# huj31415/nbody3d-webgpu

Hardware: AMD Instinct MI355X
Metric: pair-interactions/s (higher is better)
Workload: dtype f32; 1 GPU; N=262144 Plummer sphere, dt=1e-3, G=1, eps2=1e-4, i-sharded over 1 GPU(s); n=262144, kernel_variant=f32pk_symw_ipl16_j1_w2048_r32t128, parallelism=1gpu

## Files before the change

### include/nbody3d_hip.h

```cpp
#ifndef NBODY3D_HIP_H
#define NBODY3D_HIP_H

#include <stddef.h>
#include <stdint.h>

#ifdef __cplusplus
extern "C" {
#endif
#if defined(__GNUC__)
#pragma GCC visibility push(default)
#endif

#define NB_ABI_VERSION 2u
#define NB_ABI_MINOR 4u

typedef struct nb_sim nb_sim;

typedef enum nb_status {
    NB_OK = 0,
    NB_ERR_INVALID = 1,
    NB_ERR_NO_DEVICE = 2,
    NB_ERR_HIP = 3,
    NB_ERR_STATE = 4,
    NB_ERR_NOMEM = 5,
    NB_ERR_COMM = 6,
    NB_NOT_READY = 7
} nb_status;

typedef enum nb_precision { NB_F32 = 0, NB_F64 = 1 } nb_precision;

#define NB_FLAG_EXT_STREAM 1u
#define NB_FLAG_LDS_ONLY 4u
#define NB_FLAG_NO_FUSE 8u
#define NB_FLAG_POISON 16u

#define NB_FLAG_JPK_FENCED 32u

#define NB_FLAG_NO_SYM 64u

#define NB_FLAG_SYM_SHARD 128u

#define NB_FLAG_WHOLE_SWEEPS 256u

typedef enum nb_array { NB_BODIES = 0, NB_VEL = 1, NB_ACCEL = 2 } nb_array;

typedef struct nb_config {
    uint32_t struct_size;
    uint32_t n;
    uint32_t precision;
    uint32_t tile;
    double eps2;
    int32_t device;
    uint32_t shard_begin;
    uint32_t shard_count;
    void *ext_stream;
    void *ext_bodies;
    uint32_t force_variant;
    uint32_t jsplit;
    uint32_t flags;
    uint32_t layer_budget_mib;
    uint32_t reserved[4];
} nb_config;

uint32_t nb_abi_version(void);
uint32_t nb_abi_minor(void);

int nb_device_count(void);

int nb_create(const nb_config *cfg, nb_sim **out);

void nb_destroy(nb_sim *s);

int nb_upload(nb_sim *s, const void *bodies, const void *vel, const void *accel);

int nb_set_params(nb_sim *s, double dt, double G);

int nb_step(nb_sim *s, uint32_t nsteps);

int nb_download(nb_sim *s, void *bodies, void *vel, void *accel);

int nb_sync(nb_sim *s);

const char *nb_last_error(nb_sim *s);


int nb_device_ptr(nb_sim *s, int which , void **out);

typedef int (*nb_exchange_fn)(void *user, void *bodies_dev, size_t elem_size,
                              uint32_t n, uint32_t shard_begin,
                              uint32_t shard_count, void *hip_stream);
int nb_set_exchange(nb_sim *s, nb_exchange_fn fn, void *user);

typedef int (*nb_exchange_wait_fn)(void *user, void *hip_stream);
int nb_set_exchange_overlapped(nb_sim *s, nb_exchange_fn begin, nb_exchange_wait_fn wait, void *user);

// ... 80 lines not shown
```

### nbody3d-webgpu_amd/csrc/kernels/symmetric.hip.h

```cpp
#pragma once

namespace nb {

template <typename T> struct SymRowT { T x, y, z; };
using SymRow = SymRowT<float>;

constexpr uint32_t kFlushSteps = 4096;

template <int NG>
__device__ __forceinline__ void flush_resident_sums(float (*hi)[64], const int lane, const bool flushed, nb_f2 (&ax)[NG], nb_f2 (&ay)[NG], nb_f2 (&az)[NG])
{
    if (flushed) {
#pragma unroll
        for (int c = 0; c < NG; ++c) {
            hi[6 * c + 0][lane] += ax[c].x; hi[6 * c + 1][lane] += ay[c].x; hi[6 * c + 2][lane] += az[c].x;
            hi[6 * c + 3][lane] += ax[c].y; hi[6 * c + 4][lane] += ay[c].y; hi[6 * c + 5][lane] += az[c].y;
        }
    } else {
#pragma unroll
        for (int c = 0; c < NG; ++c) {
            hi[6 * c + 0][lane] = ax[c].x; hi[6 * c + 1][lane] = ay[c].x; hi[6 * c + 2][lane] = az[c].x;
            hi[6 * c + 3][lane] = ax[c].y; hi[6 * c + 4][lane] = ay[c].y; hi[6 * c + 5][lane] = az[c].y;
        }
    }
#pragma unroll
    for (int c = 0; c < NG; ++c) { ax[c] = nb_f2{0, 0}; ay[c] = nb_f2{0, 0}; az[c] = nb_f2{0, 0}; }
}

__device__ __forceinline__ float wave_rot1(float v)
{
    const int iv = __builtin_bit_cast(int, v);
    return __builtin_bit_cast(float, __builtin_amdgcn_update_dpp(iv, iv, 0x13C , 0xF, 0xF, false));
}

template <int WS, int NG, int J>
__global__ __launch_bounds__(64 * WS) __attribute__((amdgpu_waves_per_eu(NG > 4 ? 2 : 4, NG > 4 ? 2 : 4)))
void nb_force_sym(const float4* __restrict__ bodies, SymRow* __restrict__ partial, const SymPlan pl, const uint32_t n, const float eps2)
{
    constexpr uint32_t RB = 128u * NG;
    constexpr uint32_t S = RB * WS;
    constexpr uint32_t CH = 64u * J;
    constexpr uint32_t CPS = S / CH;
    __shared__ float red[WS > 1 ? 2 : 1][WS > 1 ? WS : 1][3 * J][64];
    const int tid = threadIdx.x;
    const int lane = tid & 63;
    const uint32_t w = __builtin_amdgcn_readfirstlane(tid >> 6);

    const uint32_t g = blockIdx.x / pl.q, q = blockIdx.x % pl.q;
    const uint32_t ring = (pl.H + (g < pl.n_hi ? 1u : 0u)) * CPS;
    const uint32_t total = ring + CPS;
    const uint32_t c0 = (uint32_t)(((uint64_t)q * total) / pl.q), c1 = (uint32_t)(((uint64_t)(q + 1) * total) / pl.q);

    nb_f2 xi[NG], yi[NG], zi[NG], mi[NG], ax[NG], ay[NG], az[NG];
    {
        const float4* rb = bodies + (size_t)g * S + w * RB + lane;
#pragma unroll
        for (int c = 0; c < NG; ++c) {
            const float4 b0 = ld4(rb + (2 * c) * 64), b1 = ld4(rb + (2 * c + 1) * 64);
            xi[c] = nb_f2{b0.x, b1.x}; yi[c] = nb_f2{b0.y, b1.y}; zi[c] = nb_f2{b0.z, b1.z}; mi[c] = nb_f2{b0.w, b1.w};
            ax[c] = nb_f2{0, 0}; ay[c] = nb_f2{0, 0}; az[c] = nb_f2{0, 0};
        }
    }
    const nb_f2 e2 = nb_f2{eps2, eps2};

    uint32_t done = 0;
    for (uint32_t k = c0; k < c1; ++k) {
        const bool sym = k < ring;
        const uint32_t d = k / CPS;
        uint32_t tb = g + 1 + d;
        if (tb >= pl.nsb) tb -= pl.nsb;
        const uint32_t tstart = sym ? tb * S + (k % CPS) * CH : g * S + (k - ring) * CH;
        if (tstart >= n) continue;
        float tx[J], ty[J], tz[J], tm[J];
        nb_f2 bx[J], by[J], bz[J];
#pragma unroll
        for (int u = 0; u < J; ++u) {
            const float4 t = ld4(bodies + tstart + u * 64 + lane);
            tx[u] = t.x; ty[u] = t.y; tz[u] = t.z; tm[u] = t.w;
            bx[u] = nb_f2{0, 0}; by[u] = nb_f2{0, 0}; bz[u] = nb_f2{0, 0};
        }
        for (int st = 0; st < 64; ++st) {
#pragma unroll
            for (int u = 0; u < J; ++u) {
                const nb_f2 px = nb_f2{tx[u], tx[u]}, py = nb_f2{ty[u], ty[u]}, pz = nb_f2{tz[u], tz[u]}, pm = nb_f2{tm[u], tm[u]};
#pragma unroll
// ... 53 lines not shown
#pragma unroll
                for (int u = 0; u < J; ++u) {
                    red[buf][w][3 * u + 0][lane] = bx[u].x + bx[u].y;
                    red[buf][w][3 * u + 1][lane] = by[u].x + by[u].y;
                    red[buf][w][3 * u + 2][lane] = bz[u].x + bz[u].y;
                }
                __syncthreads();
                if (w == done % WS) {
#pragma unroll
                    for (int u = 0; u < J; ++u) {
                        float sx = red[buf][0][3 * u + 0][lane], sy = red[buf][0][3 * u + 1][lane], sz = red[buf][0][3 * u + 2][lane];
#pragma unroll
                        for (int ww = 1; ww < WS; ++ww) { sx += red[buf][ww][3 * u + 0][lane]; sy += red[buf][ww][3 * u + 1][lane]; sz += red[buf][ww][3 * u + 2][lane]; }
                        out[u * 64] = SymRow{sx, sy, sz};
                    }
                }
            }
        }
    }
    SymRow* out = partial + (size_t)(pl.r_layer0 + q) * pl.np + (size_t)g * S + w * RB + lane;
#pragma unroll
    for (int c = 0; c < NG; ++c) {
        out[(2 * c) * 64] = SymRow{ax[c].x, ay[c].x, az[c].x};
        out[(2 * c + 1) * 64] = SymRow{ax[c].y, ay[c].y, az[c].y};
    }
}

struct SymWK { uint32_t np, nsb, W, total_hi, total_lo, n_hi, zc, ups, r_layer0, t_layer0; };
#define SYMW_PLAN_PARAMS const uint32_t W_, const uint32_t ups_, const uint32_t nsb_, const uint32_t zc_, const uint32_t r_layer0_, const uint32_t t_layer0_
typedef uint32_t nb_u4 __attribute__((ext_vector_type(4)));
template <int TAIL>
__device__ __forceinline__ void symw_record_and_tail(const uint32_t* rec_at, nb_u4& rec, uint32_t (&tail)[TAIL])
{
    static_assert(TAIL == 1 || TAIL == 4, "f32: eps2; f64: G, eps2");
    constexpr int kTailOffset = 4 * 8 + 6 * 4;
    if constexpr (TAIL == 1) {
        asm volatile("s_load_dwordx4 %0, %2, 0x0\n\ts_load_dword %1, %3, %4\n\ts_waitcnt lgkmcnt(0)"
                     : "=&s"(rec), "=&s"(tail[0]) : "s"(rec_at), "s"(__builtin_amdgcn_kernarg_segment_ptr()), "n"(kTailOffset) : "memory");
    } else {
        nb_u4 t;
        asm volatile("s_load_dwordx4 %0, %2, 0x0\n\ts_load_dwordx4 %1, %3, %4\n\ts_waitcnt lgkmcnt(0)"
                     : "=&s"(rec), "=&s"(t) : "s"(rec_at), "s"(__builtin_amdgcn_kernarg_segment_ptr()), "n"(kTailOffset) : "memory");
        tail[0] = t.x; tail[1] = t.y; tail[2] = t.z; tail[3] = t.w;
    }
}

__device__ __forceinline__ SymWK symw_plan_words(uint32_t S, uint32_t cps, uint32_t W, uint32_t ups, uint32_t nsb, uint32_t zc, uint32_t r_layer0, uint32_t t_layer0)
{
    const uint32_t H = (nsb - 1u) >> 1, n_hi = (nsb & 1u) ? 0u : nsb >> 1;
    const uint32_t total_lo = (H + 1u) * cps + zc, total_hi = total_lo + (n_hi ? cps : 0u);
    return SymWK{(nsb + (zc ? 1u : 0u)) * S, nsb, W, total_hi, total_lo, n_hi, zc, ups, r_layer0, t_layer0};
}

template <int NG, int J>
__global__ __launch_bounds__(256) __attribute__((amdgpu_waves_per_eu(NG >= 4 ? 2 : 4, NG > 4 ? 2 : (NG < 4 ? 8 : 4))))
void nb_force_symw(const uint32_t* __restrict__ gtab, const float4* __restrict__ bodies, SymRow* __restrict__ partial, SymRow* __restrict__ spill,
                   SYMW_PLAN_PARAMS, const float eps2_arg ,
                   uint32_t* __restrict__ queue, const uint32_t npieces, const uint32_t pieces_off)
{
    constexpr uint32_t S = 128u * NG;
    constexpr int GW = NG < 4 ? NG : 4;
    constexpr uint32_t CH = 64u * J;
    constexpr uint32_t CPS = S / CH;
    const SymWK pl = symw_plan_words(S, CPS, W_, ups_, nsb_, zc_, r_layer0_, t_layer0_);
    const int lane = threadIdx.x & 63, wi = threadIdx.x >> 6;
    const uint32_t w = __builtin_amdgcn_readfirstlane(blockIdx.x * 4u + wi);
    const bool active = w < pl.W;
    NB_STAMP(0);
    __shared__ float red[4][6 * NG][64];
    __shared__ uint32_t fin[4];
    const uint32_t ups = pl.ups, ush = (uint32_t)__builtin_ctz(ups), ustep = 64u >> ush,
                   tab1 = 2u * (pl.np / S);
    nb_u4 rec;
    uint32_t tail[1];
    symw_record_and_tail(gtab + tab1 + 4u * (active ? w : 0u), rec, tail);
    const float eps2 = __builtin_bit_cast(float, tail[0]);
    const nb_f2 e2 = nb_f2{eps2, eps2};
    const uint32_t first_lo = pl.n_hi * pl.total_hi, first_z = first_lo + (pl.nsb - pl.n_hi) * pl.total_lo;
    const uint32_t slot = rec.w;
    NB_STAMP_LIGHT(1);
    bool first_part = true;

    auto run = [&](uint32_t u, const uint32_t uend, const uint32_t piece_layer) -> uint32_t {
        uint32_t gfin = ~0u;
        while (u < uend) {
            const uint32_t p = u >> ush;
            uint32_t g, k, total;
            if (p < first_lo) { g = p / pl.total_hi; k = p - g * pl.total_hi; total = pl.total_hi; }
            else if (p < first_z) { const uint32_t r = p - first_lo; g = pl.n_hi + r / pl.total_lo; k = r - (g - pl.n_hi) * pl.total_lo; total = pl.total_lo; }
            else { g = pl.nsb; k = p - first_z; total = pl.zc; }
            const uint32_t ring = g < pl.nsb ? total - CPS - pl.zc : 0u;
            const uint32_t both_end = g < pl.nsb ? ring + pl.zc : 0u;
            uint32_t ug_end = (p - k + total) * ups;
            if (ug_end > uend) ug_end = uend;

            nb_f2 xi[NG], yi[NG], zi[NG], mi[NG], ax[NG], ay[NG], az[NG];
            {
                const float4* rb = bodies + (size_t)g * S + lane;
#pragma unroll
                for (int c = 0; c < NG; ++c) {
                    const float4 b0 = ld4(rb + (2 * c) * 64), b1 = ld4(rb + (2 * c + 1) * 64);
                    xi[c] = nb_f2{b0.x, b1.x}; yi[c] = nb_f2{b0.y, b1.y}; zi[c] = nb_f2{b0.z, b1.z}; mi[c] = nb_f2{b0.w, b1.w};
                    ax[c] = nb_f2{0, 0}; ay[c] = nb_f2{0, 0}; az[c] = nb_f2{0, 0};
                }
            }
            uint32_t since = 0;
            bool flushed = false;
            while (u < ug_end) {
                const uint32_t q0 = u & (ups - 1u);
                uint32_t nun = ups - q0;
                if (nun > ug_end - u) nun = ug_end - u;
                const uint32_t s0 = q0 * ustep, s1 = s0 + nun * ustep;
                u += nun;
                if (since >= kFlushSteps) {
                    flush_resident_sums<NG>(red[wi], lane, flushed, ax, ay, az);
                    flushed = true;
                    since = 0;
                }
                since += s1 - s0;
                const bool sym = k < both_end, zsweep = k >= ring && sym;
                const uint32_t d = k / CPS;
                uint32_t tb = g + 1 + d;
                if (tb >= pl.nsb) tb -= pl.nsb;
                const uint32_t tstart = k < ring ? tb * S + (k % CPS) * CH : zsweep ? pl.nsb * S + (k - ring) * CH : g * S + (k - both_end) * CH;
                const uint32_t zrow = g * pl.zc + (k - ring);
                ++k;
                float tx[J], ty[J], tz[J], tm[J];
                nb_f2 bx[J], by[J], bz[J];
                const uint32_t src = ((uint32_t)lane - s0) & 63u;
#pragma unroll
                for (int uu = 0; uu < J; ++uu) {
                    const float4 t = ld4(bodies + tstart + uu * 64 + src);
                    tx[uu] = t.x; ty[uu] = t.y; tz[uu] = t.z; tm[uu] = t.w;
                    bx[uu] = nb_f2{0, 0}; by[uu] = nb_f2{0, 0}; bz[uu] = nb_f2{0, 0};
                }
                auto steps = [&](auto both) {
                    constexpr bool BOTH = decltype(both)::value;
                    for (uint32_t st = s0; st < s1; ++st) {
#pragma unroll
                        for (int uu = 0; uu < J; ++uu) {
                            const nb_f2 px = nb_f2{tx[uu], tx[uu]}, py = nb_f2{ty[uu], ty[uu]}, pz = nb_f2{tz[uu], tz[uu]}, pm = nb_f2{tm[uu], tm[uu]};
#pragma unroll
                            for (int c0g = 0; c0g < NG; c0g += GW) {
                                nb_f2 dx[GW], dy[GW], dz[GW], d2[GW], r[GW], si[GW], sj[GW];
#pragma unroll
                                for (int c = 0; c < GW; ++c) dx[c] = px - xi[c0g + c];
#pragma unroll
                                for (int c = 0; c < GW; ++c) dy[c] = py - yi[c0g + c];
#pragma unroll
                                for (int c = 0; c < GW; ++c) dz[c] = pz - zi[c0g + c];
#pragma unroll
                                for (int c = 0; c < GW; ++c) d2[c] = __builtin_elementwise_fma(dx[c], dx[c], e2);
#pragma unroll
                                for (int c = 0; c < GW; ++c) d2[c] = __builtin_elementwise_fma(dy[c], dy[c], d2[c]);
#pragma unroll
                                for (int c = 0; c < GW; ++c) d2[c] = __builtin_elementwise_fma(dz[c], dz[c], d2[c]);
#pragma unroll
                                for (int c = 0; c < GW; ++c) r[c] = d2[c] * d2[c];
#pragma unroll
                                for (int c = 0; c < GW; ++c) r[c] = r[c] * d2[c];
#pragma unroll
                                for (int c = 0; c < GW; ++c) r[c] = nb_f2{nb_rsq(r[c].x), nb_rsq(r[c].y)};
#pragma unroll
                                for (int c = 0; c < GW; ++c) si[c] = pm * r[c];
                                if constexpr (BOTH) {
#pragma unroll
                                    for (int c = 0; c < GW; ++c) sj[c] = mi[c0g + c] * r[c];
                                }
#pragma unroll
                                for (int c = 0; c < GW; ++c) ax[c0g + c] = __builtin_elementwise_fma(si[c], dx[c], ax[c0g + c]);
#pragma unroll
                                for (int c = 0; c < GW; ++c) ay[c0g + c] = __builtin_elementwise_fma(si[c], dy[c], ay[c0g + c]);
#pragma unroll
                                for (int c = 0; c < GW; ++c) az[c0g + c] = __builtin_elementwise_fma(si[c], dz[c], az[c0g + c]);
                                if constexpr (BOTH) {
#pragma unroll
                                    for (int c = 0; c < GW; ++c) bx[uu] = __builtin_elementwise_fma(-sj[c], dx[c], bx[uu]);
#pragma unroll
                                    for (int c = 0; c < GW; ++c) by[uu] = __builtin_elementwise_fma(-sj[c], dy[c], by[uu]);
// ... 45 lines not shown
                        ax[c].y += red[wi][6 * c + 3][lane]; ay[c].y += red[wi][6 * c + 4][lane]; az[c].y += red[wi][6 * c + 5][lane];
                    }
                    red[wi][6 * c + 0][lane] = ax[c].x; red[wi][6 * c + 1][lane] = ay[c].x; red[wi][6 * c + 2][lane] = az[c].x;
                    red[wi][6 * c + 3][lane] = ax[c].y; red[wi][6 * c + 4][lane] = ay[c].y; red[wi][6 * c + 5][lane] = az[c].y;
                }
                break;
            }
            SymRow* out = partial + (size_t)(pl.r_layer0 + gtab[2 * g + 1] - 1u) * pl.np + (size_t)g * S + lane;
#pragma unroll
            for (int c = 0; c < NG; ++c) {
                if (flushed) {
                    ax[c].x += red[wi][6 * c + 0][lane]; ay[c].x += red[wi][6 * c + 1][lane]; az[c].x += red[wi][6 * c + 2][lane];
                    ax[c].y += red[wi][6 * c + 3][lane]; ay[c].y += red[wi][6 * c + 4][lane]; az[c].y += red[wi][6 * c + 5][lane];
                }
                out[(2 * c) * 64] = SymRow{ax[c].x, ay[c].x, az[c].x};
                out[(2 * c + 1) * 64] = SymRow{ax[c].y, ay[c].y, az[c].y};
            }
        }
        return gfin;
    };
    const uint32_t gfin = run(active ? rec.x : 0u, active ? rec.y : 0u, ~0u);
    NB_STAMP_LIGHT(8);
    if (lane == 0) fin[wi] = gfin;
    __syncthreads();
    NB_STAMP_LIGHT(9);
    if (gfin != ~0u) {
        int members = 0, mine = 0;
#pragma unroll
        for (int j = 0; j < 4; ++j) {
            const bool same = fin[j] == gfin;
            members += same;
            mine += same && j < wi;
        }
        SymRow* out = partial + (size_t)(pl.r_layer0 + rec.z) * pl.np + (size_t)gfin * S + lane;
        for (int r = mine; r < 2 * NG; r += members) {
            float sx = 0.f, sy = 0.f, sz = 0.f;
#pragma unroll
            for (int j = 0; j < 4; ++j)
                if (fin[j] == gfin) { sx += red[j][3 * r + 0][lane]; sy += red[j][3 * r + 1][lane]; sz += red[j][3 * r + 2][lane]; }
            out[r * 64] = SymRow{sx, sy, sz};
        }
    }
    if (npieces) {
        for (;;) {
            uint32_t id = 0;
            if (lane == 0) id = __hip_atomic_fetch_add(queue, 1u, __ATOMIC_RELAXED, __HIP_MEMORY_SCOPE_AGENT);
            id = __builtin_amdgcn_readfirstlane(id);
            if (id >= npieces) break;
            const uint32_t pu = gtab[pieces_off + 2u * id], ll = gtab[pieces_off + 2u * id + 1u];
            (void)run(pu, pu + (ll >> 16), ll & 0xffffu);
        }
    }
    NB_STAMP(4);
}

__device__ __forceinline__ double wave_rot1(double v)
{
    const long long b = __builtin_bit_cast(long long, v);
    const int lo = (int)(b & 0xffffffffll), hi = (int)(b >> 32);
    const unsigned rlo = (unsigned)__builtin_amdgcn_update_dpp(lo, lo, 0x13C, 0xF, 0xF, false);
    const unsigned rhi = (unsigned)__builtin_amdgcn_update_dpp(hi, hi, 0x13C, 0xF, 0xF, false);
    return __builtin_bit_cast(double, (long long)(((unsigned long long)rhi << 32) | rlo));
}

template <int IPL>
__global__ __launch_bounds__(256) __attribute__((amdgpu_waves_per_eu(2, 2)))
void nb_force_symw64(const uint32_t* __restrict__ gtab, const double4* __restrict__ bodies, SymRowT<double>* __restrict__ partial, SymRowT<double>* __restrict__ spill,
                     SYMW_PLAN_PARAMS, const double G_arg, const double eps2_arg ,
                     uint32_t* __restrict__ queue, const uint32_t npieces, const uint32_t pieces_off)
{
    constexpr uint32_t S = 64u * IPL, CH = 64u, CPS = S / CH;
    const SymWK pl = symw_plan_words(S, CPS, W_, ups_, nsb_, zc_, r_layer0_, t_layer0_);
    constexpr int GW = 4;
    const int lane = threadIdx.x & 63, wi = threadIdx.x >> 6;
    const uint32_t w = __builtin_amdgcn_readfirstlane(blockIdx.x * 4u + wi);
    const bool active = w < pl.W;
    __shared__ double red[4][3 * IPL][64];
    __shared__ uint32_t fin[4];
    const uint32_t ups = pl.ups, ush = (uint32_t)__builtin_ctz(ups), ustep = 64u >> ush,
                   tab1 = 2u * (pl.np / S);
    nb_u4 rec;
    uint32_t tail[4];
    symw_record_and_tail(gtab + tab1 + 4u * (active ? w : 0u), rec, tail);
    const double G = __builtin_bit_cast(double, (unsigned long long)tail[1] << 32 | tail[0]), eps2 = __builtin_bit_cast(double, (unsigned long long)tail[3] << 32 | tail[2]);
    const uint32_t first_lo = pl.n_hi * pl.total_hi, first_z = first_lo + (pl.nsb - pl.n_hi) * pl.total_lo;
    const uint32_t slot = rec.w;
    auto run = [&](uint32_t u, const uint32_t uend, const uint32_t piece_layer) -> uint32_t {
        uint32_t gfin = ~0u;
        while (u < uend) {
            const uint32_t p = u >> ush;
            uint32_t g, k, total;
            if (p < first_lo) { g = p / pl.total_hi; k = p - g * pl.total_hi; total = pl.total_hi; }
            else if (p < first_z) { const uint32_t r = p - first_lo; g = pl.n_hi + r / pl.total_lo; k = r - (g - pl.n_hi) * pl.total_lo; total = pl.total_lo; }
            else { g = pl.nsb; k = p - first_z; total = pl.zc; }
            const uint32_t ring = g < pl.nsb ? total - CPS - pl.zc : 0u, both_end = g < pl.nsb ? ring + pl.zc : 0u;
            uint32_t ug_end = (p - k + total) * ups;
            if (ug_end > uend) ug_end = uend;
            double xi[IPL], yi[IPL], zi[IPL], mi[IPL], ax[IPL], ay[IPL], az[IPL];
#pragma unroll
            for (int c = 0; c < IPL; ++c) {
                const double4 b = ld4(bodies + (size_t)g * S + c * 64 + lane);
                xi[c] = b.x; yi[c] = b.y; zi[c] = b.z; mi[c] = b.w * G;
                ax[c] = 0; ay[c] = 0; az[c] = 0;
            }
            while (u < ug_end) {
                const uint32_t q0 = u & (ups - 1u);
// ... 566 lines not shown
```

### nbody3d-webgpu_amd/csrc/nb_engine.hip

```cpp
#include "nb_internal.h"
#include "nb_kernels.hip.h"
#include "../../include/nbody3d_hip_plan.h"

#include <hip/hip_ext.h>

#include <algorithm>
#include <cmath>
#include <cstdio>
#include <cstdlib>
#include <cstring>
#include <new>
#include <type_traits>

namespace {
thread_local std::string g_create_error = "";
}

namespace nbi {
int fail(nb_sim* s, int code, const std::string& msg)
{
    if (s) s->err = msg; else g_create_error = msg;
    return code;
}
void set_create_error(const std::string& msg) { g_create_error = msg; }
// ... 40 lines not shown
#define NB_PK_TABLE(NAME, F)                                            \
    const void* NAME(int ng, int ls, int tl)                            \
    {                                                                    \
        if (tl == 8) {           \
            if (ng == 1) { NB_LS_CASES_T8(F, 1, ls) }                    \
            if (ng == 2) { NB_LS_CASES_T8(F, 2, ls) }                    \
            if (ng == 4) { NB_LS_CASES_T8(F, 4, ls) }                    \
        }                                                                \
        if (tl == 1) {                                                   \
            if (ng == 1) { NB_LS_CASES(F, 1, 1, ls) }                    \
            if (ng == 2) { NB_LS_CASES(F, 2, 1, ls) }                    \
            if (ng == 4) { NB_LS_CASES(F, 4, 1, ls) }                    \
        } else if (tl == 4) {                                            \
            if (ng == 1) { NB_LS_CASES_T4(F, 1, ls) }                    \
            if (ng == 2) { NB_LS_CASES_T4(F, 2, ls) }                    \
            if (ng == 4) { NB_LS_CASES_T4(F, 4, ls) }                    \
        }                                                                \
        return nullptr;                                                  \
    }
NB_PK_TABLE(pk_force_kernel, nb_force_pk)
NB_PK_TABLE(pk_fused_kernel, nb_step_fused)

template <typename T>
const void* scalar_kernel(int ipl, int ls)
{
    if (ls == 1) {
        if (ipl == 1) return (const void*)&nb::nb_force<T, 1, 1>;
        if (ipl == 2) return (const void*)&nb::nb_force<T, 2, 1>;
        if (ipl == 4) return (const void*)&nb::nb_force<T, 4, 1>;
        return nullptr;
    }
    if (ipl != 1) return nullptr;
    if (ls == 4) return (const void*)&nb::nb_force<T, 1, 4>;
    if (ls == 16) return (const void*)&nb::nb_force<T, 1, 16>;
    if (ls == 64) return (const void*)&nb::nb_force<T, 1, 64>;
    return nullptr;
}

const void* sgpr_kernel(int ipl, int ws)
{
    if (ipl == 4 && ws == 5) return (const void*)&nb::nb_force_pk_sgpr<2, 4, true>;
    if (ipl == 4) return ws == 4 ? (const void*)&nb::nb_force_pk_sgpr<2, 4> : (const void*)&nb::nb_force_pk_sgpr<2, 1>;
    if (ipl == 8 && ws == 5) return (const void*)&nb::nb_force_pk_sgpr<4, 4, true>;
    if (ipl == 8) return ws == 4 ? (const void*)&nb::nb_force_pk_sgpr<4, 4> : (const void*)&nb::nb_force_pk_sgpr<4, 1>;
    return nullptr;
}

const void* rank_kernel_of(bool f64, int ipl)
{
    if (f64) return ipl == 8 ? (const void*)&nb::nb_force_symw64_rank<8> : nullptr;
    return ipl == 16 ? (const void*)&nb::nb_force_symw_rank<8> : ipl == 8 ? (const void*)&nb::nb_force_symw_rank<4> : nullptr;
}

const void* kernel_of(bool f64, const Shape& sh)
{
    switch (sh.kind) {
        case kScalar: return f64 ? scalar_kernel<double>(sh.ipl, sh.ls) : scalar_kernel<float>(sh.ipl, sh.ls);
        case kPkLds: return f64 || (sh.ipl & 1) ? nullptr : pk_force_kernel(sh.ipl / 2, sh.ls, sh.x);
        case kFused: return f64 || (sh.ipl & 1) ? nullptr : pk_fused_kernel(sh.ipl / 2, sh.ls, sh.x);
        case kPkSgpr: return f64 || sh.ls != 1 || !(sh.x == 1 || sh.x == 4 || sh.x == 5) ? nullptr : sgpr_kernel(sh.ipl, sh.x);
        case kDirect:
            if (f64 || sh.ipl != 2 || sh.ls != 64) return nullptr;
            return sh.x == 1 ? (const void*)&nb::nb_step_direct<16> : sh.x == 2 ? (const void*)&nb::nb_step_direct<32> : nullptr;
        case kSym:
            if (sh.ls != 1) return nullptr;
            if (f64) return sh.ipl == 8 && sh.x == 3 ? (const void*)&nb::nb_force_symw64<8> : nullptr;
            if (sh.x == 4) return sh.ipl == 8 ? (const void*)&nb::nb_force_sym<4, 4, 2> : nullptr;
            if (sh.ipl == 4) return sh.x == 3 ? (const void*)&nb::nb_force_symw<2, 1> : nullptr;
            if (sh.ipl == 8) return sh.x == 1 ? (const void*)&nb::nb_force_symw<4, 2> : sh.x == 3 ? (const void*)&nb::nb_force_symw<4, 1> : nullptr;
            if (sh.ipl == 16) return sh.x == 1 ? (const void*)&nb::nb_force_symw<8, 2> : sh.x == 3 ? (const void*)&nb::nb_force_symw<8, 1> : nullptr;
            return nullptr;
        case kJpk:
            if (f64 || sh.ipl != 1 || sh.ls != 1) return nullptr;
            return sh.x == 4 ? (const void*)&nb::nb_step_jpk<4> : sh.x == 8 ? (const void*)&nb::nb_step_jpk<8>
                   : sh.x == 6 ? (const void*)&nb::nb_step_jpk<16> : nullptr;
        default: return nullptr;
    }
}

void plan_handle(nb_sim* s, const nb_config& cfg, int n_cu, double clock_hz, double device_mem)
{
    PlanInput in;
    if (device_mem > 0) in.device_mem = device_mem;
    in.n = s->n; in.sb = s->sb; in.sc = s->sc; in.f64 = s->f64; in.cfg = cfg; in.n_cu = n_cu; in.clock_hz = clock_hz;
    if (!s->no_device)
        in.occupancy = [f64 = s->f64](const Shape& sh, int block) {
            int occ = 0;
            const void* fn = kernel_of(f64, sh);
            if (!fn || hipOccupancyMaxActiveBlocksPerMultiprocessor(&occ, fn, block, 0) != hipSuccess) { (void)hipGetLastError(); return 0; }
            return occ;
        };
    LaunchPlan p = plan_launch(in);
    s->ipl = p.ipl; s->ls = p.ls; s->ws = p.ws; s->tl = p.tl;
    s->packed = p.packed; s->sgpr = p.sgpr; s->fused = p.fused; s->direct = p.direct; s->jpk = p.jpk; s->swap_acc = p.swap_acc;
    s->jsplit = p.jsplit; s->j_per_split = p.j_per_split; s->junits = p.junits; s->own_split0 = p.own_split0; s->own_splits = p.own_splits;
    s->sym = p.sym; s->symw = p.symw; s->sym_rank = p.sym_rank;
    s->sym_np = p.sym_np; s->sym_layers = p.sym_layers; s->sym_g0 = p.sym_g0; s->sym_g1 = p.sym_g1;
    static_assert(sizeof(s->sym_plan) == sizeof(p.sym_plan), "nb_sim::sym_plan mirrors LaunchPlan::sym_plan");
    memcpy(s->sym_plan, p.sym_plan, sizeof s->sym_plan);
    static_assert(sizeof(s->sym_rank_plan) == sizeof(p.sym_rank_plan), "nb_sim::sym_rank_plan mirrors LaunchPlan::sym_rank_plan");
    memcpy(s->sym_rank_plan, p.sym_rank_plan, sizeof s->sym_rank_plan);
    s->sym_passes = std::move(p.sym_passes);
    s->sym_local = p.sym_local;
    s->sym_tab_host = std::move(p.sym_tab_host);
    s->sym_spill_rows = p.sym_spill_rows;
    s->sym_pieces = p.sym_pieces;
    s->variant = std::move(p.variant);
}

Shape shape_of(const nb_sim* s)
{
    if (s->sym) return {kSym, s->ipl, 1, s->ws};
    if (s->jpk) return {kJpk, 1, 1, s->ws};
    if (s->direct) return {kDirect, s->ipl, s->ls, s->tl};
    if (s->fused) return {kFused, s->ipl, s->ls, s->tl};
    if (s->sgpr) return {kPkSgpr, s->ipl, 1, s->ws};
    if (s->packed) return {kPkLds, s->ipl, s->ls, s->tl};
    return {kScalar, s->ipl, s->ls, 1};
}

size_t sym_layer_rows(const nb_sim* s) { return s->sym_rank ? (size_t)(s->sym_g1 - s->sym_g0) * ipb_of(shape_of(s)) : (size_t)s->sym_np; }

bool streams_gm(const nb_sim* s) { return !s->f64 && s->packed && !s->jpk; }
// ... 20 lines not shown
    return NB_OK;
}

void launch_kernel(const void* fn, dim3 grid, dim3 block, void** args, hipStream_t stream, hipEvent_t t0, hipEvent_t t1)
{
    if (t0 || t1) (void)hipExtLaunchKernel(fn, grid, block, args, 0, stream, t0, t1, 0);
    else (void)hipLaunchKernel(fn, grid, block, args, 0, stream);
}

template <typename T>
void launch_force(nb_sim* s, int part = 0, hipEvent_t t0 = nullptr, hipEvent_t t1 = nullptr)
{
    using V4 = typename nb::vec4<T>::type;
    const Shape sh = shape_of(s);
    if (s->sym_rank) {
        const nbp::LaunchPlan::SymPass& ps = s->sym_passes[s->sym_pass];
        nb::SymRankPlan rp;
        memcpy(&rp, ps.plan, sizeof rp);
        uint32_t w0 = part == 2 ? rp.WA : 0u, w1 = part == 1 ? rp.WA : rp.WA + rp.WB;
        if (w1 <= w0) return;
        const void* b = jstream(s, s->cur);
        void* p = s->partial;
        const uint32_t* tab = s->sym_tab + ps.tab_off;
        uint32_t n = s->n, k_lo = ps.k_lo, k_hi = ps.k_hi, d0 = ps.d0;
        void* sp = s->sym_spill;
        if (s->f64) {
            double G = s->G, e2 = s->eps2;
            void* args[] = {&b, &p, &tab, &rp, &n, &G, &e2, &w0, &w1, &sp, &k_lo, &k_hi, &d0};
            launch_kernel(rank_kernel_of(true, sh.ipl), dim3(ceil_div(w1 - w0, 4u)), dim3(256), args, s->stream, t0, t1);
        } else {
            float e2 = (float)s->eps2;
            void* args[] = {&b, &p, &tab, &rp, &n, &e2, &w0, &w1, &sp, &k_lo, &k_hi, &d0};
            launch_kernel(rank_kernel_of(false, sh.ipl), dim3(ceil_div(w1 - w0, 4u)), dim3(256), args, s->stream, t0, t1);
        }
        return;
    }
    if (s->symw) {
        nb::SymWPlan pl;
        memcpy(&pl, s->sym_plan, sizeof pl);
        const void* b = jstream(s, s->cur);
        void* p = s->partial;
        const uint32_t* tab = s->sym_tab;
        void* sp = s->sym_spill;
        uint32_t* queue = s->sym_queue;
        uint32_t npieces = s->sym_pieces, pieces_off = 2u * (pl.np / ipb_of(sh)) + 4u * pl.W;
        if (npieces) (void)hipMemsetAsync(queue, 0, sizeof(uint32_t), s->stream);
        if (s->f64) {
            double G = s->G, e2 = s->eps2;
            void* args[] = {&tab, &b, &p, &sp, &pl.W, &pl.ups, &pl.nsb, &pl.zc, &pl.r_layer0, &pl.t_layer0, &G, &e2, &queue, &npieces, &pieces_off};
            launch_kernel(kernel_of(true, sh), dim3(ceil_div(pl.W, 4u)), dim3(256), args, s->stream, t0, t1);
        } else {
            float e2 = (float)s->eps2;
            void* args[] = {&tab, &b, &p, &sp, &pl.W, &pl.ups, &pl.nsb, &pl.zc, &pl.r_layer0, &pl.t_layer0, &e2, &queue, &npieces, &pieces_off};
            launch_kernel(kernel_of(false, sh), dim3(ceil_div(pl.W, 4u)), dim3(256), args, s->stream, t0, t1);
        }
        return;
    }
    if (s->sym) {
        nb::SymPlan pl;
        memcpy(&pl, s->sym_plan, sizeof pl);
        const float4* b = (const float4*)jstream(s, s->cur);
        nb::SymRow* p = (nb::SymRow*)s->partial;
        float e2 = (float)s->eps2;
        uint32_t n = s->n;
        void* args[] = {&b, &p, &pl, &n, &e2};
        launch_kernel(kernel_of(false, sh), dim3(pl.nsb * pl.q), dim3(64 * sh.x), args, s->stream, t0, t1);
        return;
    }
    nb::SplitWindow win{0, 0xffffffffu, 0};
    uint32_t ny = s->jsplit;
    if (part == 1) { win.base = s->own_split0; ny = s->own_splits; }
    else if (part == 2) { win.hole_begin = s->own_split0; win.hole_count = s->own_splits; ny = s->jsplit - s->own_splits; }
    if (ny == 0) return;
    dim3 grid(ceil_div(s->sc, ipb_of(sh)), ny), block(nb::kBlock);
    const V4* b = (const V4*)jstream(s, s->cur);
    V4* p = (V4*)s->partial;
    T G = (T)s->G, e2 = (T)s->eps2;
    uint32_t n = s->n, sb = s->sb, sc = s->sc, jps = s->j_per_split;
    const V4* zr = (const V4*)s->zero_row;
    void* args[] = {&b, &p, &n, &sb, &sc, &G, &e2, &jps, &win, &zr};
    launch_kernel(kernel_of(s->f64, sh), grid, block, args, s->stream, t0, t1);
}

void ensure_pairs(nb_sim* s)
{
    if (!s->jpk || (s->pairs_ok && s->pairs_G == s->G)) return;
    const float4* b = (const float4*)s->bodies[s->cur];
    float4* p = (float4*)s->pairs[s->cur];
    uint32_t n = s->n;
    float G = (float)s->G;
    void* args[] = {&b, &p, &n, &G};
    (void)hipLaunchKernel((const void*)&nb::nb_pairs_pack<0>, dim3(ceil_div(ceil_div(n, 2u), nb::kBlock)), dim3(nb::kBlock), args, 0, s->stream);
    s->pairs_ok = true; s->pairs_G = s->G;
}

void launch_jpk(nb_sim* s, hipEvent_t t0, hipEvent_t t1)
{
    const Shape sh = shape_of(s);
    dim3 grid(ceil_div(s->n, 64u), s->jsplit), block(64 * jpk_ws(sh.x));
    const float4 *bin = (const float4*)s->bodies[s->cur], *pin = (const float4*)s->pairs[s->cur];
    float4 *bout = (float4*)s->bodies[s->cur ^ 1], *pout = (float4*)s->pairs[s->cur ^ 1];
    float4 *v = (float4*)s->vel, *a = (float4*)s->acc, *part = (float4*)s->jpartial;
    uint32_t* tk = s->tickets;
    uint32_t n = s->n, upw = s->junits, poison = (s->poison ? 1u : 0u) | (s->jpk_fenced ? 2u : 0u);
    float G = (float)s->G, e2 = (float)s->eps2, dt = (float)s->dt;
    void* args[] = {&bin, &pin, &bout, &pout, &v, &a, &part, &tk, &n, &upw, &poison, &G, &e2, &dt};
    launch_kernel(kernel_of(false, sh), grid, block, args, s->stream, t0, t1);
// ... 285 lines not shown
    int count = 0;
    hipError_t e = hipGetDeviceCount(&count);
    if (e != hipSuccess || count <= 0)
        return fail(nullptr, NB_ERR_NO_DEVICE,
                    std::string("nb_create: no HIP device (") + (e != hipSuccess ? hipGetErrorString(e) : "count = 0") +
                        "); this engine has no CPU fallback");
    int dev = cfg.device;
    if (dev < 0) { if (hipGetDevice(&dev) != hipSuccess) dev = 0; }
    if (dev >= count) return fail(nullptr, NB_ERR_INVALID, "nb_create: device ordinal out of range");

    nb_sim* s = new (std::nothrow) nb_sim;
    if (!s) return fail(nullptr, NB_ERR_NOMEM, "nb_create: out of host memory");
    s->n = cfg.n; s->sb = sb; s->sc = sc;
    s->f64 = cfg.precision == NB_F64;
    s->esz = s->f64 ? 8 : 4;
    s->eps2 = eps2;
    s->device = dev;

    auto bail = [&](int code, const std::string& msg) {
        std::string m = msg;
        nb_destroy(s);
        return fail(nullptr, code, m);
    };
#define NB_HIPC(call)                                                                        \
    do {                                                                                     \
        hipError_t e_ = (call);                                                              \
        if (e_ != hipSuccess) return bail(NB_ERR_HIP, std::string(#call) + ": " + hipGetErrorString(e_)); \
    } while (0)

    NB_HIPC(hipSetDevice(dev));
    hipDeviceProp_t prop;
    NB_HIPC(hipGetDeviceProperties(&prop, dev));
    if (cfg.ext_stream || (cfg.flags & NB_FLAG_EXT_STREAM)) { s->stream = (hipStream_t)cfg.ext_stream; s->own_stream = false; }
    else { NB_HIPC(hipStreamCreateWithFlags(&s->stream, hipStreamNonBlocking)); s->own_stream = true; }

    const int n_cu = prop.multiProcessorCount > 0 ? prop.multiProcessorCount : 256;
    s->n_cu = n_cu;
    const double clock_hz = prop.clockRate > 0 ? 1e3 * prop.clockRate : 2.4e9;
    plan_handle(s, cfg, n_cu, clock_hz, (double)prop.totalGlobalMem);
    if (s->sym && (!s->sym_rank || s->sym_local) && !cfg.force_variant) {
        size_t free_b = 0, total_b = 0;
        auto need = [&]() { return 3.0 * s->esz * (double)sym_layer_rows(s) * s->sym_layers + 12.0 * s->esz * s->sym_np; };
        if (hipMemGetInfo(&free_b, &total_b) == hipSuccess && need() > 0.9 * (double)free_b) {
            nb_config fit = cfg;
            fit.layer_budget_mib = (uint32_t)std::max(1.0, 0.6 * (double)free_b / 1048576.0);
            plan_handle(s, fit, n_cu, clock_hz, (double)prop.totalGlobalMem);
            if (s->sym && need() > 0.9 * (double)free_b) {
                cfg.flags |= NB_FLAG_NO_SYM;
                plan_handle(s, cfg, n_cu, clock_hz, (double)prop.totalGlobalMem);
            }
        }
    }
    if (!kernel_of(s->f64, shape_of(s))) return bail(NB_ERR_INVALID, "nb_create: no kernel for shape " + s->variant);

    const size_t row = 4 * s->esz;
    if (cfg.ext_bodies) { s->bodies[0] = cfg.ext_bodies; s->own_bodies = false; }
    else {
        const size_t rows = s->sym ? s->sym_np : s->n;
        NB_HIPC(hipMalloc(&s->bodies[0], row * rows));
        if (s->sym) NB_HIPC(hipMemset(s->bodies[0], 0, row * rows));
        s->own_bodies = true;
        if (s->fused) NB_HIPC(hipMalloc(&s->bodies[1], row * s->n));
    }
    NB_HIPC(hipMalloc(&s->vel, row * s->sc));
    NB_HIPC(hipMalloc(&s->acc, row * s->sc));
    auto alloc_partial = [&](size_t bytes) -> hipError_t {
        if (s->partial) return hipErrorInvalidValue;
        s->partial_bytes = bytes;
        return hipMalloc(&s->partial, bytes);
    };
    if (s->sym) {
        NB_HIPC(alloc_partial((size_t)3 * s->esz * sym_layer_rows(s) * s->sym_layers));
        if (s->sym_rank) NB_HIPC(hipMalloc(&s->sym_A, 4 * s->esz * s->sym_np));
        if (s->sym_spill_rows) {
            NB_HIPC(hipMalloc(&s->sym_spill, (size_t)3 * s->esz * s->sym_spill_rows));
            NB_HIPC(hipMemset(s->sym_spill, 0, (size_t)3 * s->esz * s->sym_spill_rows));
        }
        if (s->symw && s->sym_pieces) {
            NB_HIPC(hipMalloc((void**)&s->sym_queue, 64));
            NB_HIPC(hipMemset(s->sym_queue, 0, 64));
        }
        if (s->symw) {
            NB_HIPC(hipMalloc((void**)&s->sym_tab, sizeof(uint32_t) * s->sym_tab_host.size()));
            NB_HIPC(hipMemcpy(s->sym_tab, s->sym_tab_host.data(), sizeof(uint32_t) * s->sym_tab_host.size(), hipMemcpyHostToDevice));
        }
    } else if (!s->fused) {
        NB_HIPC(alloc_partial(row * s->sc * s->jsplit));
    }
    if (s->partial_bytes != (s->sym ? (size_t)3 * s->esz * sym_layer_rows(s) * s->sym_layers : s->fused ? (size_t)0 : row * s->sc * s->jsplit))
        return bail(NB_ERR_STATE, "nb_create: the partial-sum buffer does not have the size this handle's kernels index");
    if (s->jpk) {
        const size_t pbytes = ((size_t)ceil_div(ceil_div(s->n, 2u), 4u) + 3) * 128;
        const uint32_t iblocks = ceil_div(s->n, 64u);
        for (auto& p : s->pairs) { NB_HIPC(hipMalloc(&p, pbytes)); NB_HIPC(hipMemset(p, 0, pbytes)); }
        NB_HIPC(hipMalloc((void**)&s->tickets, sizeof(uint32_t) * iblocks));
        NB_HIPC(hipMemset(s->tickets, 0, sizeof(uint32_t) * iblocks));
        if (s->jsplit > 1) {
            NB_HIPC(hipMalloc(&s->jpartial, (size_t)16 * 64 * iblocks * s->jsplit));
            NB_HIPC(hipMemset(s->jpartial, 0xff, (size_t)16 * 64 * iblocks * s->jsplit));
        }
        NB_HIPC(hipDeviceSynchronize());
        s->poison = (cfg.flags & NB_FLAG_POISON) != 0;
        s->jpk_fenced = (cfg.flags & NB_FLAG_JPK_FENCED) != 0;
    }
    NB_HIPC(hipMalloc(&s->zero_row, 64));
    NB_HIPC(hipMemsetAsync(s->zero_row, 0, 64, s->stream));
// ... 665 lines not shown
```

### nbody3d-webgpu_amd/csrc/nb_internal.h

```cpp
#pragma once
#include "../../include/nbody3d_hip.h"
#include "nb_plan.h"

#include <hip/hip_runtime.h>

#include <cstdint>
#include <string>
#include <vector>

struct nb_events { hipEvent_t e[8]; bool two, xchg, rs; };

struct nb_rccl;

struct nb_frame_slot {
    float* h_bodies = nullptr;
    float* h_speed = nullptr;
    float* d_bodies = nullptr;
    float* d_speed = nullptr;
    hipEvent_t packed = nullptr;
    hipEvent_t landed = nullptr;
    uint64_t step = 0;
    bool in_flight = false, valid = false;
};

struct nb_sim {
    uint32_t n = 0, sb = 0, sc = 0;
    bool f64 = false;
    size_t esz = 4;
    int device = 0;
    bool no_device = false;
    double eps2 = 1e-4;
    hipStream_t stream = nullptr;
    bool own_stream = false;
    void* bodies[2] = {nullptr, nullptr};
    int cur = 0;
    bool own_bodies = false;
    void* gm[2] = {nullptr, nullptr};
    bool gm_ok = false;
    double gm_G = 0.0;
    void* vel = nullptr;
    void* acc = nullptr;
    void* partial = nullptr;
    size_t partial_bytes = 0;
    double* diag = nullptr;
    void* zero_row = nullptr;
    uint32_t diag_blocks = 0, diag_chunk = 256;
    double dt = 0.0, G = 0.0;
    bool params_set = false, uploaded = false;
    uint64_t steps_done = 0;
    int ipl = 1, ls = 1;
    bool packed = false;
    bool sgpr = false;
    int ws = 1;
    int tl = 1;
    bool fused = false;
    bool direct = false;
    bool jpk = false;
    void* pairs[2] = {nullptr, nullptr};
    bool pairs_ok = false;
    double pairs_G = 0.0;
    void* jpartial = nullptr;
    uint32_t* tickets = nullptr;
    uint32_t junits = 0;
    bool poison = false;
    bool jpk_fenced = false;
    int acc_parity = 0;
    bool swap_acc = false;
    uint32_t jsplit = 1, j_per_split = 0;
    bool sym = false;
    uint32_t sym_np = 0, sym_layers = 0;
    uint32_t sym_plan[16] = {0};
    bool symw = false;
    uint32_t* sym_tab = nullptr;
    std::vector<uint32_t> sym_tab_host;
    void* sym_spill = nullptr;
    uint32_t sym_spill_rows = 0;
    uint32_t sym_pieces = 0;
    uint32_t* sym_queue = nullptr;
    bool sym_rank = false;
    uint32_t sym_g0 = 0, sym_g1 = 0;
    uint32_t sym_rank_plan[16] = {0};
    std::vector<nbp::LaunchPlan::SymPass> sym_passes;
    uint32_t sym_pass = 0;
    bool sym_local = false;
    void* sym_A = nullptr;
    std::string variant, err;
    nb_exchange_fn xfn = nullptr;
    nb_exchange_wait_fn xwait = nullptr;
    void* xuser = nullptr;
    bool gather_pending = false;
    uint32_t own_split0 = 0, own_splits = 0;
    nb_rccl* rccl = nullptr;
    bool timing = false;
    struct graph_slot {
        hipGraph_t graph = nullptr;
        hipGraphExec_t exec = nullptr;
        double dt = 0.0, G = 0.0;
        int parity = 0;
    } graphs[2];
    bool graphs_ok = true;
    std::vector<nb_events> pool;
    std::vector<nb_events> pending;
    size_t pool_next = 0;
    hipStream_t frame_stream = nullptr;
    static constexpr int kFrameSlots = 4;
    nb_frame_slot frame[kFrameSlots];
    int frame_next = 0;
    int frame_latest = -1;
    int n_cu = 256;
    struct field_buf { void* p = nullptr; size_t cap = 0; } fld_pts, fld_acc, fld_phi, fld_part;
};

namespace nbi {

int fail(nb_sim* s, int code, const std::string& msg);
void set_create_error(const std::string& msg);
const std::string& create_error();

int rccl_exchange_begin(nb_sim* s);
int rccl_reduce_scatter_A(nb_sim* s);
int sym_rank_phase_a(nb_sim* s, void* after_force = nullptr, bool split_at_gather = false, nb_events* stamps = nullptr);
int sym_rank_phase_b(nb_sim* s);
int rccl_exchange_wait(nb_sim* s);
bool rccl_overlapped(const nb_sim* s);
void rccl_release(nb_sim* s);

}
```

### nbody3d-webgpu_amd/nbody3d_amd/capi.py

```python
import ctypes as C
import os

import numpy as np

_PKG = os.path.dirname(os.path.abspath(__file__))
_LIB_PATH = os.environ.get("NB_ENGINE_LIB") or os.path.normpath(os.path.join(_PKG, "..", "csrc", "libnbody3d_hip.so"))

NB_F32, NB_F64 = 0, 1
NB_FLAG_EXT_STREAM = 1
NB_FLAG_LDS_ONLY = 4
NB_FLAG_NO_FUSE = 8
NB_FLAG_POISON = 16
NB_FLAG_JPK_FENCED = 32
NB_FLAG_NO_SYM = 64
NB_FLAG_SYM_SHARD = 128
NB_FLAG_WHOLE_SWEEPS = 256
NB_RCCL_ID_BYTES = 128
NB_RCCL_OVERLAP = 1
NB_MULTI_PEER, NB_MULTI_RCCL, NB_MULTI_PEER_OVERLAP = 0, 1, 2
NB_NOT_READY = 7
NB_FIELD_AT_BODIES, NB_FIELD_F64, NB_FIELD_DEVICE = 1, 2, 4
STATUS = {0: "NB_OK", 1: "NB_ERR_INVALID", 2: "NB_ERR_NO_DEVICE", 3: "NB_ERR_HIP",
          4: "NB_ERR_STATE", 5: "NB_ERR_NOMEM", 6: "NB_ERR_COMM", 7: "NB_NOT_READY"}
ABI_VERSION = 2
ABI_MINOR = 3


class NBodyError(RuntimeError):
    def __init__(self, code, msg):
        super().__init__("%s: %s" % (STATUS.get(code, code), msg))
        self.code = code


class nb_config(C.Structure):
    _fields_ = [
        ("struct_size", C.c_uint32), ("n", C.c_uint32), ("precision", C.c_uint32), ("tile", C.c_uint32),
        ("eps2", C.c_double), ("device", C.c_int32), ("shard_begin", C.c_uint32), ("shard_count", C.c_uint32),
        ("ext_stream", C.c_void_p), ("ext_bodies", C.c_void_p),
        ("force_variant", C.c_uint32), ("jsplit", C.c_uint32), ("flags", C.c_uint32), ("layer_budget_mib", C.c_uint32),
        ("reserved", C.c_uint32 * 4),
    ]


class nb_plan_info(C.Structure):
    _fields_ = [("struct_size", C.c_uint32)] + [(k, C.c_uint32) for k in (
        "kind", "ipl", "ls", "x", "jsplit", "j_per_split", "own_split0", "own_splits",
        "sym", "symw", "sym_rank", "sym_np", "sym_layers", "sym_g0", "sym_g1")] + [
        ("sym_plan", C.c_uint32 * 11), ("tab_len", C.c_uint32), ("variant", C.c_char * 112),
        ("sym_ups", C.c_uint32), ("sym_spill_rows", C.c_uint32), ("sym_rank_plan", C.c_uint32 * 16),
        ("sym_pass", C.c_uint32), ("sym_passes", C.c_uint32), ("sym_pass_k_lo", C.c_uint32), ("sym_pass_k_hi", C.c_uint32),
        ("sym_pass_d0", C.c_uint32), ("sym_local", C.c_uint32)]


class nb_step_timing(C.Structure):
    _fields_ = [("struct_size", C.c_uint32), ("launches", C.c_uint32), ("force_ms", C.c_double), ("sym_reduce_ms", C.c_double),
                ("reduce_scatter_ms", C.c_double), ("integrate_ms", C.c_double), ("allgather_ms", C.c_double),
                ("span_ms", C.c_double), ("reduce_scatters", C.c_uint32), ("allgathers", C.c_uint32)]


class nb_field_request(C.Structure):
    _fields_ = [("struct_size", C.c_uint32), ("m", C.c_uint32), ("flags", C.c_uint32), ("first_body", C.c_uint32),
                ("points", C.c_void_p), ("accel", C.c_void_p), ("phi", C.c_void_p)]


EXCHANGE_FN = C.CFUNCTYPE(C.c_int, C.c_void_p, C.c_void_p, C.c_size_t, C.c_uint32, C.c_uint32, C.c_uint32, C.c_void_p)
EXCHANGE_WAIT_FN = C.CFUNCTYPE(C.c_int, C.c_void_p, C.c_void_p)

SYMBOLS = ["nb_abi_version", "nb_device_count", "nb_create", "nb_destroy", "nb_upload", "nb_set_params", "nb_step",
           "nb_download", "nb_sync", "nb_last_error", "nb_device_ptr", "nb_set_exchange",
# ... 574 lines not shown
```

Baseline: 6735 billion pair-interactions/s.

## Pair two symmetric sweeps per lane using packed f32 with swapped halves

Adds a paired-sweep path for the symmetric-walk force kernel with J=1. Two traveler chunks are loaded into the two halves of packed float2 registers and processed together, so the resident i-bodies are compared against both at once using packed math and lane swaps. The reaction sums are accumulated with fused DPP rotate-add instructions instead of a separate rotate and add. The paired path becomes the default for ipl 8/16 with x=3, and a new flag restores single sweeps; the cost is higher register pressure and more complex sweep bookkeeping.

Result: faster. 6826 billion pair-interactions/s (median of 6 runs) (+1.4%).

```diff
diff --git a/include/nbody3d_hip.h b/include/nbody3d_hip.h
--- a/include/nbody3d_hip.h
+++ b/include/nbody3d_hip.h
@@ -41,6 +41,8 @@
 #define NB_FLAG_SYM_SHARD 128u
 
 #define NB_FLAG_WHOLE_SWEEPS 256u
+
+#define NB_FLAG_SINGLE_SWEEPS 512u
 
 typedef enum nb_array { NB_BODIES = 0, NB_VEL = 1, NB_ACCEL = 2 } nb_array;
 
diff --git a/nbody3d-webgpu_amd/csrc/kernels/symmetric.hip.h b/nbody3d-webgpu_amd/csrc/kernels/symmetric.hip.h
--- a/nbody3d-webgpu_amd/csrc/kernels/symmetric.hip.h
+++ b/nbody3d-webgpu_amd/csrc/kernels/symmetric.hip.h
@@ -31,6 +31,19 @@
 {
     const int iv = __builtin_bit_cast(int, v);
     return __builtin_bit_cast(float, __builtin_amdgcn_update_dpp(iv, iv, 0x13C , 0xF, 0xF, false));
+}
+
+__device__ __forceinline__ void wave_rot1_add(float& r, float s)
+{
+    asm("v_add_f32_dpp %0, %0, %1 wave_ror:1 row_mask:0xf bank_mask:0xf" : "+v"(r) : "v"(s));
+}
+
+__device__ __forceinline__ nb_f2 symw_swap(nb_f2 v) { return __builtin_shufflevector(v, v, 1, 0); }
+__device__ __forceinline__ nb_f2 symw_sub(int cross, nb_f2 t, nb_f2 res) { return (cross ? symw_swap(t) : t) - res; }
+__device__ __forceinline__ nb_f2 symw_mul(int cross, nb_f2 t, nb_f2 r) { return (cross ? symw_swap(t) : t) * r; }
+__device__ __forceinline__ nb_f2 symw_fnma(int cross, nb_f2 s, nb_f2 d, nb_f2 acc)
+{
+    return cross ? __builtin_elementwise_fma(-symw_swap(s), symw_swap(d), acc) : __builtin_elementwise_fma(-s, d, acc);
 }
 
 template <int WS, int NG, int J>
@@ -190,12 +203,11 @@
     return SymWK{(nsb + (zc ? 1u : 0u)) * S, nsb, W, total_hi, total_lo, n_hi, zc, ups, r_layer0, t_layer0};
 }
 
-template <int NG, int J>
-__global__ __launch_bounds__(256) __attribute__((amdgpu_waves_per_eu(NG >= 4 ? 2 : 4, NG > 4 ? 2 : (NG < 4 ? 8 : 4))))
-void nb_force_symw(const uint32_t* __restrict__ gtab, const float4* __restrict__ bodies, SymRow* __restrict__ partial, SymRow* __restrict__ spill,
-                   SYMW_PLAN_PARAMS, const float eps2_arg ,
-                   uint32_t* __restrict__ queue, const uint32_t npieces, const uint32_t pieces_off)
-{
+template <int NG, int J, bool PAIR>
+__device__ __forceinline__ void symw_sweeps(const uint32_t* __restrict__ gtab, const float4* __restrict__ bodies, SymRow* __restrict__ partial, SymRow* __restrict__ spill,
+                                            SYMW_PLAN_PARAMS, uint32_t* __restrict__ queue, const uint32_t npieces, const uint32_t pieces_off)
+{
+    static_assert(!PAIR || J == 1, "paired sweeps: one traveler per lane and sweep");
     constexpr uint32_t S = 128u * NG;
     constexpr int GW = NG < 4 ? NG : 4;
     constexpr uint32_t CH = 64u * J;
@@ -246,16 +258,18 @@
             bool flushed = false;
             while (u < ug_end) {
                 const uint32_t q0 = u & (ups - 1u);
+                bool pair = false;
+                if constexpr (PAIR) pair = q0 == 0u && ug_end - u >= 2u * ups && k + 1u < both_end;
                 uint32_t nun = ups - q0;
                 if (nun > ug_end - u) nun = ug_end - u;
                 const uint32_t s0 = q0 * ustep, s1 = s0 + nun * ustep;
-                u += nun;
+                u += pair ? 2u * ups : nun;
                 if (since >= kFlushSteps) {
                     flush_resident_sums<NG>(red[wi], lane, flushed, ax, ay, az);
                     flushed = true;
                     since = 0;
                 }
-                since += s1 - s0;
+                since += pair ? 128u : s1 - s0;
                 const bool sym = k < both_end, zsweep = k >= ring && sym;
                 const uint32_t d = k / CPS;
                 uint32_t tb = g + 1 + d;
@@ -263,6 +277,77 @@
                 const uint32_t tstart = k < ring ? tb * S + (k % CPS) * CH : zsweep ? pl.nsb * S + (k - ring) * CH : g * S + (k - both_end) * CH;
                 const uint32_t zrow = g * pl.zc + (k - ring);
                 ++k;
+                if constexpr (PAIR) {
+                    if (pair) {
+                        const bool zsweep1 = k >= ring;
+                        const uint32_t d1 = k / CPS;
+                        uint32_t tb1 = g + 1 + d1;
+                        if (tb1 >= pl.nsb) tb1 -= pl.nsb;
+                        const uint32_t tstart1 = zsweep1 ? pl.nsb * S + (k - ring) * CH : tb1 * S + (k % CPS) * CH;
+                        const uint32_t zrow1 = g * pl.zc + (k - ring);
+                        ++k;
+                        const float4 t0 = ld4(bodies + tstart + lane), t1 = ld4(bodies + tstart1 + lane);
+                        nb_f2 tx = nb_f2{t0.x, t1.x}, ty = nb_f2{t0.y, t1.y}, tz = nb_f2{t0.z, t1.z}, tm = nb_f2{t0.w, t1.w};
+                        float bx0 = 0, bx1 = 0, by0 = 0, by1 = 0, bz0 = 0, bz1 = 0;
+                        if (first_part) NB_STAMP(2);
+                        for (uint32_t st = 0; st < 64u; ++st) {
+                            nb_f2 sx = nb_f2{0, 0}, sy = nb_f2{0, 0}, sz = nb_f2{0, 0};
+#pragma unroll
+                            for (int c0g = 0; c0g < NG; c0g += GW) {
+#pragma unroll
+                                for (int f = 0; f < 2; ++f) {
+                                    nb_f2 dx[GW], dy[GW], dz[GW], d2[GW], r[GW], si[GW], sj[GW];
+#pragma unroll
+                                    for (int c = 0; c < GW; ++c) dx[c] = symw_sub(f, tx, xi[c0g + c]);
+#pragma unroll
+                                    for (int c = 0; c < GW; ++c) dy[c] = symw_sub(f, ty, yi[c0g + c]);
+#pragma unroll
+                                    for (int c = 0; c < GW; ++c) dz[c] = symw_sub(f, tz, zi[c0g + c]);
+#pragma unroll
+                                    for (int c = 0; c < GW; ++c) d2[c] = __builtin_elementwise_fma(dx[c], dx[c], e2);
+#pragma unroll
+                                    for (int c = 0; c < GW; ++c) d2[c] = __builtin_elementwise_fma(dy[c], dy[c], d2[c]);
+#pragma unroll
+                                    for (int c = 0; c < GW; ++c) d2[c] = __builtin_elementwise_fma(dz[c], dz[c], d2[c]);
+#pragma unroll
+                                    for (int c = 0; c < GW; ++c) r[c] = d2[c] * d2[c];
+#pragma unroll
+                                    for (int c = 0; c < GW; ++c) r[c] = r[c] * d2[c];
+#pragma unroll
+                                    for (int c = 0; c < GW; ++c) r[c] = nb_f2{nb_rsq(r[c].x), nb_rsq(r[c].y)};
+#pragma unroll
+                                    for (int c = 0; c < GW; ++c) si[c] = symw_mul(f, tm, r[c]);
+#pragma unroll
+                                    for (int c = 0; c < GW; ++c) sj[c] = mi[c0g + c] * r[c];
+#pragma unroll
+                                    for (int c = 0; c < GW; ++c) ax[c0g + c] = __builtin_elementwise_fma(si[c], dx[c], ax[c0g + c]);
+#pragma unroll
+                                    for (int c = 0; c < GW; ++c) ay[c0g + c] = __builtin_elementwise_fma(si[c], dy[c], ay[c0g + c]);
+#pragma unroll
+                                    for (int c = 0; c < GW; ++c) az[c0g + c] = __builtin_elementwise_fma(si[c], dz[c], az[c0g + c]);
+#pragma unroll
+                                    for (int c = 0; c < GW; ++c) sx = symw_fnma(f, sj[c], dx[c], sx);
+#pragma unroll
+                                    for (int c = 0; c < GW; ++c) sy = symw_fnma(f, sj[c], dy[c], sy);
+#pragma unroll
+                                    for (int c = 0; c < GW; ++c) sz = symw_fnma(f, sj[c], dz[c], sz);
+                                }
+                            }
+                            tx = nb_f2{wave_rot1(tx.x), wave_rot1(tx.y)}; ty = nb_f2{wave_rot1(ty.x), wave_rot1(ty.y)};
+                            tz = nb_f2{wave_rot1(tz.x), wave_rot1(tz.y)}; tm = nb_f2{wave_rot1(tm.x), wave_rot1(tm.y)};
+                            wave_rot1_add(bx0, sx.x); wave_rot1_add(bx1, sx.y); wave_rot1_add(by0, sy.x); wave_rot1_add(by1, sy.y);
+                            wave_rot1_add(bz0, sz.x); wave_rot1_add(bz1, sz.y);
+                            __builtin_amdgcn_sched_barrier(0);
+                        }
+                        if (first_part) { NB_STAMP_LIGHT(3); first_part = false; }
+                        const uint32_t home = ((uint32_t)lane + 1u) & 63u;
+                        SymRow* out0 = (zsweep ? spill + (size_t)zrow * CH : partial + (size_t)(pl.t_layer0 + d) * pl.np + tstart) + home;
+                        SymRow* out1 = (zsweep1 ? spill + (size_t)zrow1 * CH : partial + (size_t)(pl.t_layer0 + d1) * pl.np + tstart1) + home;
+                        *out0 = SymRow{bx0, by0, bz0};
+                        *out1 = SymRow{bx1, by1, bz1};
+                        continue;
+                    }
+                }
                 float tx[J], ty[J], tz[J], tm[J];
                 nb_f2 bx[J], by[J], bz[J];
                 const uint32_t src = ((uint32_t)lane - s0) & 63u;
@@ -414,6 +499,23 @@
         }
     }
     NB_STAMP(4);
+}
+
+#define SYMW_KERNEL_PARAMS const uint32_t* __restrict__ gtab, const float4* __restrict__ bodies, SymRow* __restrict__ partial, SymRow* __restrict__ spill, \
+                           SYMW_PLAN_PARAMS, const float eps2_arg ,                       \
+                           uint32_t* __restrict__ queue, const uint32_t npieces, const uint32_t pieces_off
+#define SYMW_KERNEL_ARGS gtab, bodies, partial, spill, W_, ups_, nsb_, zc_, r_layer0_, t_layer0_, queue, npieces, pieces_off
+template <int NG, int J>
+__global__ __launch_bounds__(256) __attribute__((amdgpu_waves_per_eu(NG >= 4 ? 2 : 4, NG > 4 ? 2 : (NG < 4 ? 8 : 4))))
+void nb_force_symw(SYMW_KERNEL_PARAMS)
+{
+    symw_sweeps<NG, J, false>(SYMW_KERNEL_ARGS);
+}
+template <int NG>
+__global__ __launch_bounds__(256) __attribute__((amdgpu_waves_per_eu(2, NG > 4 ? 2 : 4)))
+void nb_force_symw_pairs(SYMW_KERNEL_PARAMS)
+{
+    symw_sweeps<NG, 1, true>(SYMW_KERNEL_ARGS);
 }
 
 __device__ __forceinline__ double wave_rot1(double v)
diff --git a/nbody3d-webgpu_amd/csrc/nb_engine.hip b/nbody3d-webgpu_amd/csrc/nb_engine.hip
--- a/nbody3d-webgpu_amd/csrc/nb_engine.hip
+++ b/nbody3d-webgpu_amd/csrc/nb_engine.hip
@@ -116,7 +116,7 @@
     return ipl == 16 ? (const void*)&nb::nb_force_symw_rank<8> : ipl == 8 ? (const void*)&nb::nb_force_symw_rank<4> : nullptr;
 }
 
-const void* kernel_of(bool f64, const Shape& sh)
+const void* kernel_of(bool f64, const Shape& sh, bool single_sweeps = false)
 {
     switch (sh.kind) {
         case kScalar: return f64 ? scalar_kernel<double>(sh.ipl, sh.ls) : scalar_kernel<float>(sh.ipl, sh.ls);
@@ -131,8 +131,10 @@
             if (f64) return sh.ipl == 8 && sh.x == 3 ? (const void*)&nb::nb_force_symw64<8> : nullptr;
             if (sh.x == 4) return sh.ipl == 8 ? (const void*)&nb::nb_force_sym<4, 4, 2> : nullptr;
             if (sh.ipl == 4) return sh.x == 3 ? (const void*)&nb::nb_force_symw<2, 1> : nullptr;
-            if (sh.ipl == 8) return sh.x == 1 ? (const void*)&nb::nb_force_symw<4, 2> : sh.x == 3 ? (const void*)&nb::nb_force_symw<4, 1> : nullptr;
-            if (sh.ipl == 16) return sh.x == 1 ? (const void*)&nb::nb_force_symw<8, 2> : sh.x == 3 ? (const void*)&nb::nb_force_symw<8, 1> : nullptr;
+            if (sh.ipl == 8 && sh.x == 3) return single_sweeps ? (const void*)&nb::nb_force_symw<4, 1> : (const void*)&nb::nb_force_symw_pairs<4>;
+            if (sh.ipl == 16 && sh.x == 3) return single_sweeps ? (const void*)&nb::nb_force_symw<8, 1> : (const void*)&nb::nb_force_symw_pairs<8>;
+            if (sh.ipl == 8) return sh.x == 1 ? (const void*)&nb::nb_force_symw<4, 2> : nullptr;
+            if (sh.ipl == 16) return sh.x == 1 ? (const void*)&nb::nb_force_symw<8, 2> : nullptr;
             return nullptr;
         case kJpk:
             if (f64 || sh.ipl != 1 || sh.ls != 1) return nullptr;
@@ -259,7 +261,7 @@
         } else {
             float e2 = (float)s->eps2;
             void* args[] = {&tab, &b, &p, &sp, &pl.W, &pl.ups, &pl.nsb, &pl.zc, &pl.r_layer0, &pl.t_layer0, &e2, &queue, &npieces, &pieces_off};
-            launch_kernel(kernel_of(false, sh), dim3(ceil_div(pl.W, 4u)), dim3(256), args, s->stream, t0, t1);
+            launch_kernel(kernel_of(false, sh, s->single_sweeps), dim3(ceil_div(pl.W, 4u)), dim3(256), args, s->stream, t0, t1);
         }
         return;
     }
@@ -651,6 +653,7 @@
         }
     }
     if (!kernel_of(s->f64, shape_of(s))) return bail(NB_ERR_INVALID, "nb_create: no kernel for shape " + s->variant);
+    s->single_sweeps = (cfg.flags & NB_FLAG_SINGLE_SWEEPS) != 0;
 
     const size_t row = 4 * s->esz;
     if (cfg.ext_bodies) { s->bodies[0] = cfg.ext_bodies; s->own_bodies = false; }
diff --git a/nbody3d-webgpu_amd/csrc/nb_internal.h b/nbody3d-webgpu_amd/csrc/nb_internal.h
--- a/nbody3d-webgpu_amd/csrc/nb_internal.h
+++ b/nbody3d-webgpu_amd/csrc/nb_internal.h
@@ -76,6 +76,7 @@
     void* sym_spill = nullptr;
     uint32_t sym_spill_rows = 0;
     uint32_t sym_pieces = 0;
+    bool single_sweeps = false;
     uint32_t* sym_queue = nullptr;
     bool sym_rank = false;
     uint32_t sym_g0 = 0, sym_g1 = 0;
diff --git a/nbody3d-webgpu_amd/nbody3d_amd/capi.py b/nbody3d-webgpu_amd/nbody3d_amd/capi.py
--- a/nbody3d-webgpu_amd/nbody3d_amd/capi.py
+++ b/nbody3d-webgpu_amd/nbody3d_amd/capi.py
@@ -15,6 +15,7 @@
 NB_FLAG_NO_SYM = 64
 NB_FLAG_SYM_SHARD = 128
 NB_FLAG_WHOLE_SWEEPS = 256
+NB_FLAG_SINGLE_SWEEPS = 512
 NB_RCCL_ID_BYTES = 128
 NB_RCCL_OVERLAP = 1
 NB_MULTI_PEER, NB_MULTI_RCCL, NB_MULTI_PEER_OVERLAP = 0, 1, 2
```
